# ronghanghu/vit_10b_fsdp_example

Hardware: NVIDIA H100
Metric: vit10b images/sec (device-timed, max over ranks) (higher is better)
Workload: dtype bf16

## Files before the change

vit_10b_fsdp_example_b200/csrc/bindings.cpp:

```cpp
#include <ATen/cuda/CUDAContext.h>
#include <c10/cuda/CUDAGuard.h>
#include <torch/extension.h>

#include <cmath>
#include <optional>
#include <vector>

#include "attention_sm90.h"
#include "comm.h"
#include "elementwise.h"
#include "gemm_sm90.h"

namespace {

using torch::Tensor;
using OptT = std::optional<Tensor>;

inline const __nv_bfloat16* bf16_ptr(const Tensor& t) {
    TORCH_CHECK(t.is_cuda(), "expected a CUDA tensor");
    TORCH_CHECK(t.scalar_type() == at::kBFloat16, "expected a bf16 tensor");
    return reinterpret_cast<const __nv_bfloat16*>(t.data_ptr());
}
inline __nv_bfloat16* bf16_mut(Tensor& t) { return const_cast<__nv_bfloat16*>(bf16_ptr(t)); }
inline float* f32_ptr(const Tensor& t) {
    TORCH_CHECK(t.is_cuda() && t.scalar_type() == at::kFloat, "expected a CUDA fp32 tensor");
    return reinterpret_cast<float*>(t.data_ptr());
}
inline cudaStream_t cur_stream() { return at::cuda::getCurrentCUDAStream().stream(); }

void gemm(Tensor a, int64_t lda, int64_t major_a, Tensor b, int64_t ldb, int64_t major_b, Tensor d, int64_t ldd,
          int64_t M, int64_t N, int64_t K, OptT bias, OptT residual, int64_t ld_res, int64_t res_row_mod, OptT aux_in,
          int64_t ld_aux, OptT aux_out, int64_t ld_aux_out, OptT colsum, int64_t colsum_bi_stride, int64_t act,
          std::vector<int64_t> batch, int64_t block_n, int64_t max_ctas, std::vector<int64_t> ag) {
    c10::cuda::CUDAGuard guard(a.device());
    b200::GemmOperand A, B, D, X;
    A.ptr = bf16_ptr(a), A.ld = lda;
    B.ptr = bf16_ptr(b), B.ld = ldb;
    D.ptr = bf16_ptr(d), D.ld = ldd;
    if (!batch.empty()) {
        TORCH_CHECK(batch.size() == 8, "batch spec must have 8 entries");
        A.nb_inner = B.nb_inner = D.nb_inner = batch[0];
        A.nb_outer = B.nb_outer = D.nb_outer = batch[1];
        A.stride_b_inner = batch[2], A.stride_b_outer = batch[3];
        B.stride_b_inner = batch[4], B.stride_b_outer = batch[5];
        D.stride_b_inner = batch[6], D.stride_b_outer = batch[7];
    }
    b200::GemmEpilogue e;
    if (bias.has_value()) e.bias = bf16_ptr(*bias);
    if (residual.has_value()) e.residual = bf16_ptr(*residual), e.ld_res = ld_res, e.res_row_mod = (int)res_row_mod;
    if (aux_in.has_value()) e.aux_in = bf16_ptr(*aux_in), e.ld_aux = ld_aux;
    if (colsum.has_value()) e.colsum = f32_ptr(*colsum), e.colsum_bi_stride = colsum_bi_stride;
    e.act = static_cast<int>(act);
    if (aux_out.has_value()) {
        X = D;
        X.ptr = bf16_ptr(*aux_out), X.ld = ld_aux_out;
        e.has_aux_out = 1;
    }
    b200::GemmAgFuse fuse;
    if (!ag.empty()) {
        TORCH_CHECK(ag.size() >= 6 && (int64_t)ag.size() == 6 + ag[0] && ag[0] <= 16, "bad AG-fusion spec");
        fuse.world = (int)ag[0], fuse.rank = (int)ag[1], fuse.rows_per_slab = (int)ag[2], fuse.slab_bytes = ag[3];
        fuse.dst = reinterpret_cast<void*>(ag[4]);
        fuse.flags = reinterpret_cast<uint32_t*>(ag[5]);
        for (int64_t r = 0; r < ag[0]; ++r) fuse.peer_src[r] = static_cast<uint64_t>(ag[6 + r]);
    }
    b200::gemm_bf16(A, (int)major_a, B, (int)major_b, D, aux_out.has_value() ? &X : nullptr, (int)M, (int)N, (int)K, e,
                    (int)block_n, (int)max_ctas, cur_stream(), ag.empty() ? nullptr : &fuse);
}

void layernorm_fwd(Tensor x, Tensor gamma, Tensor beta, Tensor y, Tensor mean, Tensor rstd, double eps) {
    c10::cuda::CUDAGuard guard(x.device());
    const int D = (int)x.size(-1);
    const int rows = (int)(x.numel() / D);
    b200::layernorm_fwd(bf16_ptr(x), bf16_ptr(gamma), bf16_ptr(beta), bf16_mut(y), f32_ptr(mean), f32_ptr(rstd), rows,
                        D, (float)eps, cur_stream());
}

void layernorm_bwd(Tensor dy, Tensor x, Tensor gamma, Tensor mean, Tensor rstd, OptT dres, Tensor dx, Tensor dgamma,
                   Tensor dbeta, OptT dxsum) {
    c10::cuda::CUDAGuard guard(x.device());
    const int D = (int)x.size(-1);
    const int rows = (int)(x.numel() / D);
    b200::layernorm_bwd(bf16_ptr(dy), bf16_ptr(x), bf16_ptr(gamma), f32_ptr(mean), f32_ptr(rstd),
                        dres.has_value() ? bf16_ptr(*dres) : nullptr, bf16_mut(dx), f32_ptr(dgamma), f32_ptr(dbeta),
                        dxsum.has_value() ? f32_ptr(*dxsum) : nullptr, rows, D, cur_stream());
}

void softmax_fwd(Tensor s, int64_t rows, int64_t n, int64_t ld, double scale) {
    c10::cuda::CUDAGuard guard(s.device());
    b200::softmax_fwd(bf16_mut(s), rows, (int)n, ld, (float)scale, cur_stream());
}
void softmax_bwd(Tensor dp, Tensor p, int64_t rows, int64_t n, int64_t ld, double scale) {
    c10::cuda::CUDAGuard guard(p.device());
    b200::softmax_bwd(bf16_mut(dp), bf16_ptr(p), rows, (int)n, ld, (float)scale, cur_stream());
}

bool attention_supported(int64_t N, int64_t hd) { return b200::attention_supported((int)N, (int)hd); }

void attention_fwd(Tensor qkv, Tensor out, OptT lse, OptT probs, int64_t B, int64_t N, int64_t H, int64_t hd) {
    c10::cuda::CUDAGuard guard(qkv.device());
    TORCH_CHECK(qkv.dim() == 2 && qkv.stride(1) == 1 && out.is_contiguous(), "attention_fwd: bad layouts");
    TORCH_CHECK(!lse.has_value() || (lse->is_contiguous() && lse->numel() == B * H * N), "attention_fwd: bad lse");
    b200::attention_fwd(bf16_ptr(qkv), qkv.stride(0), bf16_mut(out), lse.has_value() ? f32_ptr(*lse) : nullptr,
                        probs.has_value() ? bf16_mut(*probs) : nullptr, probs.has_value() ? probs->size(2) : 0, (int)B,
                        (int)N, (int)H, (int)hd, cur_stream());
}

void attention_bwd(Tensor qkv, Tensor dout, Tensor out, Tensor lse, Tensor delta, Tensor dqkv, OptT colsum, int64_t B,
                   int64_t N, int64_t H, int64_t hd) {
    c10::cuda::CUDAGuard guard(qkv.device());
    TORCH_CHECK(qkv.dim() == 2 && qkv.stride(1) == 1 && dout.stride(1) == 1 && out.stride(1) == 1 &&
                    dqkv.is_contiguous() && lse.is_contiguous() && delta.is_contiguous(),
                "attention_bwd: bad layouts");
    TORCH_CHECK(lse.numel() == B * H * N && delta.numel() == B * H * N && dqkv.size(1) == 3 * H * hd,
                "attention_bwd: bad shapes");
    b200::attention_bwd(bf16_ptr(qkv), qkv.stride(0), bf16_ptr(dout), dout.stride(0), bf16_ptr(out), out.stride(0),
                        f32_ptr(lse), f32_ptr(delta), bf16_mut(dqkv), (int)B, (int)N, (int)H, (int)hd, cur_stream(),
                        colsum.has_value() ? f32_ptr(*colsum) : nullptr);
}

void cross_entropy(Tensor logits, Tensor target, OptT dlogits, Tensor loss, OptT correct) {
    c10::cuda::CUDAGuard guard(logits.device());
    TORCH_CHECK(target.scalar_type() == at::kLong && target.is_cuda(), "target must be a CUDA int64 tensor");
    const int B = (int)logits.size(0), C = (int)logits.size(1);
    b200::cross_entropy(bf16_ptr(logits), reinterpret_cast<const int64_t*>(target.data_ptr()),
                        dlogits.has_value() ? bf16_mut(*dlogits) : nullptr, f32_ptr(loss),
                        correct.has_value() ? reinterpret_cast<int*>(correct->data_ptr()) : nullptr, B, C,
                        cur_stream());
}

void im2col(Tensor img, Tensor cols, int64_t P) {
    c10::cuda::CUDAGuard guard(img.device());
    TORCH_CHECK(img.is_contiguous() && img.dim() == 4 && img.size(1) == 3, "images must be contiguous [B,3,S,S]");
    const bool is_bf16 = img.scalar_type() == at::kBFloat16;
    TORCH_CHECK(is_bf16 || img.scalar_type() == at::kFloat, "images must be fp32 or bf16");
    b200::im2col(img.data_ptr(), is_bf16, bf16_mut(cols), (int)img.size(0), (int)img.size(2), (int)P,
                 (int)cols.size(1), cur_stream());
}

void gelu_fwd(Tensor u, Tensor g) {
    c10::cuda::CUDAGuard guard(u.device());
    b200::gelu_fwd(bf16_ptr(u), bf16_mut(g), u.numel(), cur_stream());
}
void dropout(Tensor x, Tensor y, double p, int64_t key) {
    c10::cuda::CUDAGuard guard(x.device());
    TORCH_CHECK(x.is_contiguous() && y.is_contiguous() && x.numel() == y.numel(), "dropout: contiguous, same size");
    b200::dropout(bf16_ptr(x), bf16_mut(y), x.numel(), (float)p, (uint64_t)key, cur_stream());
}
void meanpool_fwd(Tensor xn, Tensor pooled, int64_t B, int64_t N) {
    c10::cuda::CUDAGuard guard(xn.device());
    TORCH_CHECK(xn.is_contiguous() && pooled.is_contiguous() && xn.numel() == pooled.numel() * N, "meanpool: bad shapes");
    b200::meanpool_fwd(bf16_ptr(xn), bf16_mut(pooled), (int)B, (int)N, (int)(pooled.numel() / B), cur_stream());
// ... 70 lines not shown
void ce_all_gather(std::vector<int64_t> src_ptrs, std::vector<int64_t> dst_ptrs, std::vector<int64_t> nbytes) {
    TORCH_CHECK(src_ptrs.size() == dst_ptrs.size() && src_ptrs.size() == nbytes.size(), "ce_all_gather: ragged lists");
    cudaStream_t stream = cur_stream();
    for (size_t i = 0; i < src_ptrs.size(); ++i) {
        cudaError_t err = cudaMemcpyAsync(reinterpret_cast<void*>(dst_ptrs[i]), reinterpret_cast<const void*>(src_ptrs[i]),
                                          static_cast<size_t>(nbytes[i]), cudaMemcpyDeviceToDevice, stream);
        TORCH_CHECK(err == cudaSuccess, "ce_all_gather: ", cudaGetErrorString(err));
    }
}
bool make_adam(const OptT& hi, const OptT& lo, const OptT& m, const OptT& v, const std::vector<double>& hyper,
               b200::AdamFuse& a) {
    if (!hi.has_value()) return false;
    TORCH_CHECK(lo.has_value() && m.has_value() && v.has_value() && hyper.size() == 6, "bad fused-AdamW arguments");
    TORCH_CHECK(hi->scalar_type() == at::kBFloat16 && lo->scalar_type() == at::kShort, "hi: bf16, lo: int16");
    a.hi = reinterpret_cast<uint16_t*>(hi->data_ptr());
    a.lo = reinterpret_cast<int16_t*>(lo->data_ptr());
    a.m = f32_ptr(*m);
    a.v = f32_ptr(*v);
    a.lr = (float)hyper[0], a.beta1 = (float)hyper[1], a.beta2 = (float)hyper[2], a.eps = (float)hyper[3];
    a.wd = (float)hyper[4];
    a.inv_bc1 = 1.f / (1.f - powf(a.beta1, (float)hyper[5]));
    a.inv_bc2 = 1.f / (1.f - powf(a.beta2, (float)hyper[5]));
    return true;
}
inline uint32_t* seq_ptr(const OptT& t) {
    if (!t.has_value()) return nullptr;
    TORCH_CHECK(t->is_cuda() && t->scalar_type() == at::kInt, "sequence counters: CUDA int32 tensor");
    return reinterpret_cast<uint32_t*>(t->data_ptr());
}
bool make_sync(const std::vector<int64_t>& sync, const std::vector<int64_t>& flag_ptrs, const OptT& seq_dev,
               const OptT& cta_ctr, b200::CommSync& cs) {
    if (sync.empty()) return false;
    TORCH_CHECK(sync.size() == 5 && seq_dev.has_value() && cta_ctr.has_value(), "bad collective sync arguments");
    cs.flag_ptrs = flag_ptrs;
    cs.rank = (int)sync[0], cs.world = (int)sync[1], cs.slot_ready = (int)sync[2], cs.slot_done = (int)sync[3];
    cs.counter_idx = (int)sync[4];
    cs.seq_dev = seq_ptr(seq_dev);
    cs.cta_ctr = seq_ptr(cta_ctr);
    return true;
}
void reduce_scatter(std::vector<int64_t> peer_ptrs, int64_t mc_ptr, int64_t rank, int64_t world, Tensor out,
                    Tensor seg_table, int64_t total_chunks, bool in_is_bf16, double scale, OptT sumsq_out,
                    int64_t max_ctas, std::vector<int64_t> sync, std::vector<int64_t> flag_ptrs, OptT seq_dev,
                    OptT cta_ctr, OptT hi, OptT lo, OptT m, OptT v, std::vector<double> hyper) {
    c10::cuda::CUDAGuard guard(out.device());
    b200::AdamFuse a;
    const bool fused = make_adam(hi, lo, m, v, hyper, a);
    b200::CommSync cs;
    const bool synced = make_sync(sync, flag_ptrs, seq_dev, cta_ctr, cs);
    b200::reduce_scatter(peer_ptrs, mc_ptr, (int)rank, (int)world, f32_ptr(out), seg_ptr(seg_table),
                         (int)seg_table.size(0), total_chunks, in_is_bf16, (float)scale,
                         sumsq_out.has_value() ? f32_ptr(*sumsq_out) : nullptr, (int)max_ctas, cur_stream(),
                         synced ? &cs : nullptr, fused ? &a : nullptr);
}
void all_reduce_mean(std::vector<int64_t> peer_ptrs, int64_t mc_ptr, int64_t rank, int64_t world, Tensor buf,
                     int64_t max_ctas, std::vector<int64_t> sync, std::vector<int64_t> flag_ptrs, OptT seq_dev,
                     OptT cta_ctr) {
    c10::cuda::CUDAGuard guard(buf.device());
    TORCH_CHECK(buf.scalar_type() == at::kBFloat16 && buf.is_contiguous(), "all_reduce_mean: contiguous bf16 buffer");
    b200::CommSync cs;
    TORCH_CHECK(make_sync(sync, flag_ptrs, seq_dev, cta_ctr, cs), "all_reduce_mean needs the flag protocol");
    b200::all_reduce_mean_bf16(peer_ptrs, mc_ptr, (int)rank, (int)world, buf.numel() * 2, 1.0f / (float)world,
                               (int)max_ctas, cur_stream(), &cs);
}
void signal_barrier(std::vector<int64_t> flag_ptrs, int64_t rank, int64_t world, int64_t slot, int64_t seq,
                    OptT seq_dev) {
    b200::signal_barrier(flag_ptrs, (int)rank, (int)world, (int)slot, (uint32_t)seq, cur_stream(), seq_ptr(seq_dev));
}
void allreduce_scalars(std::vector<int64_t> flag_ptrs, std::vector<int64_t> scratch_ptrs, int64_t rank, int64_t world,
                       int64_t slot, int64_t seq, Tensor vals, int64_t op, OptT seq_dev, int64_t counter_idx) {
    c10::cuda::CUDAGuard guard(vals.device());
    b200::allreduce_scalars(flag_ptrs, scratch_ptrs, (int)rank, (int)world, (int)slot, (uint32_t)seq, f32_ptr(vals),
                            (int)vals.numel(), (int)op, cur_stream(), seq_ptr(seq_dev), (int)counter_idx);
}
int64_t ag_chunk_bytes() { return b200::ag_chunk_bytes(); }
int64_t rs_chunk_elems() { return b200::rs_chunk_elems(); }
int64_t rs_chunk_vecs() { return b200::rs_chunk_vecs(); }

}

PYBIND11_MODULE(TORCH_EXTENSION_NAME, m) {
    m.doc() = "vit_10b_fsdp_example_b200 native sm_90a kernels";
    m.def("gemm", &gemm);
    m.def("layernorm_fwd", &layernorm_fwd);
    m.def("layernorm_bwd", &layernorm_bwd);
    m.def("softmax_fwd", &softmax_fwd);
    m.def("softmax_bwd", &softmax_bwd);
    m.def("attention_fwd", &attention_fwd);
    m.def("attention_supported", &attention_supported);
    m.def("attention_bwd", &attention_bwd);
    m.def("cross_entropy", &cross_entropy);
    m.def("im2col", &im2col);
    m.def("gelu_fwd", &gelu_fwd);
    m.def("dgelu_mul", &dgelu_mul);
    m.def("dropout", &dropout);
    m.def("meanpool_fwd", &meanpool_fwd);
    m.def("meanpool_bwd", &meanpool_bwd);
    m.def("colsum", &colsum);
    m.def("sumsq", &sumsq);
    m.def("adamw_split", &adamw_split);
    m.def("adamw_fp32", &adamw_fp32);
    m.def("split_fp32", &split_fp32);
    m.def("merge_fp32", &merge_fp32);
    m.def("clip_coef", &clip_coef);
    m.def("p2p_all_gather", &p2p_all_gather);
    m.def("ce_all_gather", &ce_all_gather);
    m.def("reduce_scatter", &reduce_scatter);
    m.def("all_reduce_mean", &all_reduce_mean);
    m.def("rs_chunk_vecs", &rs_chunk_vecs);
    m.def("signal_barrier", &signal_barrier);
    m.def("allreduce_scalars", &allreduce_scalars);
    m.def("ag_chunk_bytes", &ag_chunk_bytes);
    m.def("rs_chunk_elems", &rs_chunk_elems);
}
```

vit_10b_fsdp_example_b200/csrc/gemm_sm90.cu:

```cuda
#include <cuda.h>
#include <cuda_runtime.h>
#include <cuda_bf16.h>
#include <cstdint>
#include <cstdio>
#include <cstdlib>
#include <cstring>
#include <mutex>
#include <stdexcept>
#include <string>
#include <algorithm>
#include <unordered_map>

#include "gemm_sm90.h"
#include "ptx.cuh"
#include "wgmma.cuh"

namespace b200 {

namespace {

constexpr int kBlockM = 128;
constexpr int kBlockK = 64;
constexpr int kMmaK = 16;
constexpr int kConsumerWgs = 2;
constexpr int kNumThreads = 384;
constexpr int kEpiThreads = 128;
constexpr int kCdBufs = 4;
constexpr int kCdBufBytes = 64 * 128;

struct KernelParams {
    int M, N, K;
    int batch, nb_inner;
    int m_tiles, n_tiles;
    int n_rot;
    int group_n;
    GemmEpilogue epi;
    GemmAgFuse ag;
};

constexpr int kAgChunkBytes = 16384;

__device__ __forceinline__ uint4 ld_peer_v4(const void* ptr) {
    uint4 r;
    asm volatile("ld.global.L1::no_allocate.v4.u32 {%0, %1, %2, %3}, [%4];"
                 : "=r"(r.x), "=r"(r.y), "=r"(r.z), "=r"(r.w)
                 : "l"(ptr)
                 : "memory");
    return r;
}
__device__ __forceinline__ void red_release_gpu_add(uint32_t* ptr, uint32_t v) {
    asm volatile("red.release.gpu.global.add.u32 [%0], %1;" ::"l"(ptr), "r"(v) : "memory");
}
__device__ __forceinline__ uint32_t ld_acquire_gpu(const uint32_t* ptr) {
    uint32_t v;
    asm volatile("ld.acquire.gpu.global.u32 %0, [%1];" : "=r"(v) : "l"(ptr) : "memory");
    return v;
}
__device__ __forceinline__ void fence_proxy_async_all() { asm volatile("fence.proxy.async;" ::: "memory"); }

__device__ __forceinline__ float erf_as(float z, float& e) {
    const float az = fabsf(z);
    const float t = __frcp_rn(fmaf(0.3275911f, az, 1.0f));
    e = __expf(-az * az);
    float poly = fmaf(1.061405429f, t, -1.453152027f);
    poly = fmaf(poly, t, 1.421413741f);
    poly = fmaf(poly, t, -0.284496736f);
    poly = fmaf(poly, t, 0.254829592f);
    const float y = 1.0f - poly * t * e;
    return copysignf(y, z);
}
__device__ __forceinline__ float gelu_erf(float x) {
    float e;
    return 0.5f * x * (1.0f + erf_as(x * 0.70710678118654752f, e));
}
__device__ __forceinline__ float dgelu_erf(float x) {
    float e;
    const float cdf = 0.5f * (1.0f + erf_as(x * 0.70710678118654752f, e));
    return fmaf(x * 0.3989422804014327f, e, cdf);
}

template <int kMajorA, int kMajorB, int BLOCK_N, int kStages>
__global__ void __launch_bounds__(kNumThreads, 1)
    gemm_bf16_sm90_kernel(const __grid_constant__ CUtensorMap tmap_a, const __grid_constant__ CUtensorMap tmap_b,
                          const __grid_constant__ CUtensorMap tmap_d, const __grid_constant__ CUtensorMap tmap_aux,
                          const KernelParams p) {
    constexpr int kABytes = kBlockM * kBlockK * 2;
    constexpr int kBBytes = BLOCK_N * kBlockK * 2;
    constexpr int kStageBytes = kABytes + kBBytes;
    static_assert(BLOCK_N % 64 == 0 && BLOCK_N <= 256, "epilogue works in 64-column chunks; wgmma N <= 256");
    static_assert(kABytes % 1024 == 0 && kBBytes % 1024 == 0, "swizzle-128B needs 1024 B aligned stages");

    extern __shared__ __align__(1024) uint8_t smem[];
    uint8_t* smem_cd = smem;
    uint8_t* smem_a = smem + kCdBufs * kCdBufBytes;
    uint8_t* smem_b = smem_a + kStages * kABytes;
    uint64_t* full_bar = reinterpret_cast<uint64_t*>(smem_b + kStages * kBBytes);
    uint64_t* empty_bar = full_bar + kStages;

    const uint32_t warp_idx = threadIdx.x / 32;
    const uint32_t lane = lane_id();
    const uint32_t wg = warp_idx / 4;
    if (threadIdx.x == 0 && (smem_u32(smem) & 1023u) != 0) {
        printf("[b200] gemm: dynamic shared memory is not 1024-byte aligned\n");
        __trap();
    }

    if (warp_idx == 0 && elect_one()) {
        prefetch_tmap(&tmap_a);
        prefetch_tmap(&tmap_b);
        prefetch_tmap(&tmap_d);
        if (p.epi.has_aux_out) prefetch_tmap(&tmap_aux);
        for (int i = 0; i < kStages; ++i) {
            mbar_init(&full_bar[i], 1);
            mbar_init(&empty_bar[i], kConsumerWgs * 4);
        }
        fence_mbar_init();
    }
    __syncthreads();

    const int tiles_per_batch = p.m_tiles * p.n_tiles;
    const int total_tiles = tiles_per_batch * p.batch;
    const int num_kb = (p.K + kBlockK - 1) / kBlockK;
    const int kGroupN = p.group_n;

    auto decode_tile = [&](int t, int& b, int& mt, int& nt) {
        b = t / tiles_per_batch;
        const int r = t - b * tiles_per_batch;
        const int per_group = p.m_tiles * kGroupN;
        const int g = r / per_group;
        const int first_n = g * kGroupN;
        const int gsz = min(kGroupN, p.n_tiles - first_n);
        const int in_g = r - g * per_group;
        mt = in_g / gsz;
        nt = first_n + in_g % gsz;
        nt += p.n_rot;
        if (nt >= p.n_tiles) nt -= p.n_tiles;
    };
    const int ag_chunks_per_slab =
        p.ag.world > 1 ? static_cast<int>((p.ag.slab_bytes + kAgChunkBytes - 1) / kAgChunkBytes) : 0;

    if (wg == 0) {
        reg_dealloc<56>();
        if (warp_idx == 0) {
            if (elect_one()) {
                uint32_t stage = 0, phase = 0;
                for (int t = blockIdx.x; t < total_tiles; t += gridDim.x) {
                    int b, mt, nt;
                    decode_tile(t, b, mt, nt);
                    const int bi = b % p.nb_inner, bo = b / p.nb_inner;
                    const int m_idx = mt * kBlockM;
                    const int n_idx = nt * BLOCK_N;
                    if (p.ag.world > 1) {
                        const int last_row = min(n_idx + BLOCK_N, p.N) - 1;
                        if (last_row >= n_idx) {
                            const int s_lo = min(n_idx / p.ag.rows_per_slab, p.ag.world - 1);
                            const int s_hi = min(last_row / p.ag.rows_per_slab, p.ag.world - 1);
                            for (int sl = s_lo; sl <= s_hi; ++sl) {
                                uint32_t spins = 0;
                                while (ld_acquire_gpu(p.ag.flags + sl) < static_cast<uint32_t>(ag_chunks_per_slab)) {
                                    if (++spins > (1u << 26)) {
                                        printf("[b200] AG-fused GEMM: slab %d never arrived (block %d)\n", sl, blockIdx.x);
                                        __trap();
                                    }
                                }
                            }
                            fence_proxy_async_all();
                        }
                    }
                    for (int kb = 0; kb < num_kb; ++kb) {
                        mbar_wait(&empty_bar[stage], phase ^ 1);
                        const int k_idx = kb * kBlockK;
                        uint8_t* sa = smem_a + stage * kABytes;
                        uint8_t* sb = smem_b + stage * kBBytes;
                        mbar_arrive_expect_tx(&full_bar[stage], kStageBytes);
                        if constexpr (kMajorA == 0) {
                            tma_load_4d(&tmap_a, &full_bar[stage], sa, k_idx, m_idx, bi, bo);
                        } else {
#pragma unroll
                            for (int i = 0; i < kBlockM / 64; ++i)
                                tma_load_4d(&tmap_a, &full_bar[stage], sa + i * (64 * kBlockK * 2), m_idx + i * 64,
                                                 k_idx, bi, bo);
                        }
                        if constexpr (kMajorB == 0) {
                            tma_load_4d(&tmap_b, &full_bar[stage], sb, k_idx, n_idx, bi, bo);
                        } else {
#pragma unroll
                            for (int i = 0; i < BLOCK_N / 64; ++i)
                                tma_load_4d(&tmap_b, &full_bar[stage], sb + i * (64 * kBlockK * 2), n_idx + i * 64,
                                                 k_idx, bi, bo);
                        }
                        stage = (stage + 1 == kStages) ? 0 : stage + 1;
                        phase ^= (stage == 0);
                    }
                }
            }
        } else if (warp_idx == 1) {
            if (p.ag.world > 1) {
                const int total_chunks = p.ag.world * ag_chunks_per_slab;
                uint32_t* chunk_counter = p.ag.flags + p.ag.world;
                for (;;) {
                    int c = 0;
                    if (lane == 0) c = static_cast<int>(atomicAdd(chunk_counter, 1u));
                    c = __shfl_sync(0xffffffffu, c, 0);
                    if (c >= total_chunks) break;
                    const int k = c / ag_chunks_per_slab;
                    const int sl = (p.ag.rank + k) % p.ag.world;
                    const int64_t off = static_cast<int64_t>(c - k * ag_chunks_per_slab) * kAgChunkBytes;
                    const int64_t nbytes = min(static_cast<int64_t>(kAgChunkBytes), p.ag.slab_bytes - off);
                    const uint8_t* src = reinterpret_cast<const uint8_t*>(p.ag.peer_src[sl]) + off;
                    uint8_t* dst = static_cast<uint8_t*>(p.ag.dst) + static_cast<int64_t>(sl) * p.ag.slab_bytes + off;
                    const int nvec = static_cast<int>(nbytes / 16);
                    int i = lane;
                    for (; i + 3 * 32 < nvec; i += 4 * 32) {
                        uint4 v[4];
#pragma unroll
                        for (int u = 0; u < 4; ++u) v[u] = ld_peer_v4(src + static_cast<int64_t>(i + u * 32) * 16);
#pragma unroll
                        for (int u = 0; u < 4; ++u) *reinterpret_cast<uint4*>(dst + static_cast<int64_t>(i + u * 32) * 16) = v[u];
                    }
                    for (; i < nvec; i += 32) *reinterpret_cast<uint4*>(dst + static_cast<int64_t>(i) * 16) = ld_peer_v4(src + static_cast<int64_t>(i) * 16);
                    __threadfence();
                    __syncwarp();
                    if (lane == 0) red_release_gpu_add(p.ag.flags + sl, 1);
                }
            }
        }
    } else {
        reg_alloc<224>();
        const uint32_t cw = wg - 1;
        const uint32_t etid = threadIdx.x & 127;
        const uint32_t wrow = (warp_idx & 3) * 16 + lane / 4;
        const uint32_t cpair = (lane & 3) * 2;
        const uint32_t bar_id = 1 + cw;
        uint8_t* const grp_buf = smem_cd + cw * 2 * kCdBufBytes;
        const GemmEpilogue& e = p.epi;
        const bool ext_is_aux = e.act == kActDGelu;
        constexpr uint32_t kLbo = kBlockK * 128;
        constexpr uint32_t kKStepA = kMajorA == 0 ? (kMmaK * 2) : (kMmaK * 128);
        constexpr uint32_t kKStepB = kMajorB == 0 ? (kMmaK * 2) : (kMmaK * 128);
        constexpr uint32_t kSlabA = 64 * kBlockK * 2;
        uint32_t stage = 0, phase = 0;
        uint32_t flip = 0;
        float d[BLOCK_N / 2];

        for (int t = blockIdx.x; t < total_tiles; t += gridDim.x) {
            int b, mt, nt;
            decode_tile(t, b, mt, nt);
            const int bi = b % p.nb_inner, bo = b / p.nb_inner;
            const int m0 = mt * kBlockM + cw * 64;
            const int n0 = nt * BLOCK_N;

            uint32_t prev_stage = 0;
            for (int kb = 0; kb < num_kb; ++kb) {
                mbar_wait(&full_bar[stage], phase);
                const uint32_t a_addr = smem_u32(smem_a + stage * kABytes) + cw * kSlabA;
                const uint32_t b_addr = smem_u32(smem_b + stage * kBBytes);
                wgmma_fence();
#pragma unroll
                for (int k = 0; k < kBlockK / kMmaK; ++k) {
                    const uint64_t da = make_wgmma_desc(a_addr + k * kKStepA, kLbo, 1024, 1);
                    const uint64_t db = make_wgmma_desc(b_addr + k * kKStepB, kLbo, 1024, 1);
                    WgmmaSS<BLOCK_N, kMajorA, kMajorB>::mma(d, da, db, (kb > 0 || k > 0) ? 1u : 0u);
                }
                wgmma_commit();
                if (kb > 0) {
                    wgmma_wait<1>();
                    if (lane == 0) mbar_arrive(&empty_bar[prev_stage]);
                }
                prev_stage = stage;
                stage = (stage + 1 == kStages) ? 0 : stage + 1;
                phase ^= (stage == 0);
            }
            wgmma_wait<0>();
            if (lane == 0) mbar_arrive(&empty_bar[prev_stage]);

            const int row0 = m0 + static_cast<int>(wrow), row1 = row0 + 8;
            const bool row0_ok = row0 < p.M, row1_ok = row1 < p.M;
            const __nv_bfloat16 *ext0 = nullptr, *ext1 = nullptr;
            if (ext_is_aux) {
                ext0 = e.aux_in + static_cast<int64_t>(row0) * e.ld_aux;
                ext1 = e.aux_in + static_cast<int64_t>(row1) * e.ld_aux;
            } else if (e.residual != nullptr) {
                ext0 = e.residual + static_cast<int64_t>(e.res_row_mod > 0 ? row0 % e.res_row_mod : row0) * e.ld_res;
                ext1 = e.residual + static_cast<int64_t>(e.res_row_mod > 0 ? row1 % e.res_row_mod : row1) * e.ld_res;
            }
#pragma unroll
            for (int c = 0; c < BLOCK_N / 64; ++c) {
                const int ncol0 = n0 + c * 64;
                if (ncol0 >= p.N) continue;
                uint8_t* buf0 = grp_buf + (e.has_aux_out ? 0 : (flip & 1)) * kCdBufBytes;
                uint8_t* buf1 = grp_buf + kCdBufBytes;
                if (etid == 0) {
                    if (e.has_aux_out)
                        tma_store_wait_read<0>();
                    else
                        tma_store_wait_read<1>();
                }
                named_bar_sync(bar_id, kEpiThreads);
#pragma unroll
                for (int j = 0; j < 8; ++j) {
                    const int col = ncol0 + j * 8 + static_cast<int>(cpair);
                    const bool c0_ok = col < p.N, c1_ok = col + 1 < p.N;
                    float v[4] = {d[(c * 8 + j) * 4], d[(c * 8 + j) * 4 + 1], d[(c * 8 + j) * 4 + 2], d[(c * 8 + j) * 4 + 3]};
                    uint32_t x0 = 0, x1 = 0;
                    if (ext0 != nullptr && c0_ok) {
                        if (row0_ok) x0 = __ldg(reinterpret_cast<const uint32_t*>(ext0 + col));
                        if (row1_ok) x1 = __ldg(reinterpret_cast<const uint32_t*>(ext1 + col));
                    }
                    if (e.bias != nullptr && c0_ok) {
                        const uint32_t bw = __ldg(reinterpret_cast<const uint32_t*>(e.bias + col));
                        v[0] += bf16_lo(bw), v[1] += bf16_hi(bw), v[2] += bf16_lo(bw), v[3] += bf16_hi(bw);
                    }
                    const uint32_t off0 = wrow * 128 + ((j ^ (wrow & 7)) * 16) + cpair * 2;
                    const uint32_t off1 = off0 + 8 * 128;
                    if (e.has_aux_out) {
                        st_shared_b32(smem_u32(buf1) + off0, pack_bf16x2(v[0], v[1]));
                        st_shared_b32(smem_u32(buf1) + off1, pack_bf16x2(v[2], v[3]));
                    }
                    if (e.act == kActGelu) {
#pragma unroll
                        for (int q = 0; q < 4; ++q) v[q] = gelu_erf(v[q]);
                    } else if (ext_is_aux) {
                        v[0] *= dgelu_erf(bf16_lo(x0)), v[1] *= dgelu_erf(bf16_hi(x0));
                        v[2] *= dgelu_erf(bf16_lo(x1)), v[3] *= dgelu_erf(bf16_hi(x1));
                    }
                    if (e.residual != nullptr && !ext_is_aux) {
                        v[0] += bf16_lo(x0), v[1] += bf16_hi(x0), v[2] += bf16_lo(x1), v[3] += bf16_hi(x1);
                    }
                    if (!(row0_ok && c0_ok)) v[0] = 0.f;
                    if (!(row0_ok && c1_ok)) v[1] = 0.f;
                    if (!(row1_ok && c0_ok)) v[2] = 0.f;
                    if (!(row1_ok && c1_ok)) v[3] = 0.f;
                    st_shared_b32(smem_u32(buf0) + off0, pack_bf16x2(v[0], v[1]));
                    st_shared_b32(smem_u32(buf0) + off1, pack_bf16x2(v[2], v[3]));
                }
                fence_proxy_async_smem();
                named_bar_sync(bar_id, kEpiThreads);
                if (etid == 0) {
                    tma_store_4d(&tmap_d, buf0, ncol0, m0, bi, bo);
                    tma_store_commit();
                    if (e.has_aux_out) {
                        tma_store_4d(&tmap_aux, buf1, ncol0, m0, bi, bo);
                        tma_store_commit();
                    }
                }
                if (e.colsum != nullptr) {
                    const int ccol = etid & 63;
                    const int rhalf = etid >> 6;
                    const int jj = ccol >> 3, within = ccol & 7;
                    float s = 0.f;
#pragma unroll 8
                    for (int r = 0; r < 32; ++r) {
                        const int rr = rhalf * 32 + r;
                        const uint8_t* ptr = buf0 + rr * 128 + ((jj ^ (rr & 7)) * 16) + within * 2;
                        s += __bfloat162float(*reinterpret_cast<const __nv_bfloat16*>(ptr));
                    }
                    if (ncol0 + ccol < p.N)
                        atomicAdd(e.colsum + static_cast<int64_t>(bi) * e.colsum_bi_stride + ncol0 + ccol, s);
                }
                ++flip;
            }
        }
        if (etid == 0) tma_store_wait<0>();
    }
}

using EncodeFn = CUresult (*)(CUtensorMap*, CUtensorMapDataType, cuuint32_t, void*, const cuuint64_t*,
                              const cuuint64_t*, const cuuint32_t*, const cuuint32_t*, CUtensorMapInterleave,
                              CUtensorMapSwizzle, CUtensorMapL2promotion, CUtensorMapFloatOOBfill);

EncodeFn get_encode_fn() {
    static EncodeFn fn = nullptr;
    static std::once_flag once;
    std::call_once(once, [] {
        void* sym = nullptr;
        cudaDriverEntryPointQueryResult qres;
        cudaError_t err = cudaGetDriverEntryPoint("cuTensorMapEncodeTiled", &sym, cudaEnableDefault, &qres);
        if (err != cudaSuccess || qres != cudaDriverEntryPointSuccess || sym == nullptr)
            throw std::runtime_error("cuTensorMapEncodeTiled not available from the driver");
        fn = reinterpret_cast<EncodeFn>(sym);
    });
    return fn;
}

struct TmapKey {
    uint64_t ptr;
    int64_t d[4];
    int64_t s[3];
    int32_t box[2];
    bool operator==(const TmapKey& o) const { return std::memcmp(this, &o, sizeof(TmapKey)) == 0; }
};
struct TmapKeyHash {
    size_t operator()(const TmapKey& k) const {
        const uint64_t* w = reinterpret_cast<const uint64_t*>(&k);
        size_t h = 1469598103934665603ull;
        for (size_t i = 0; i < sizeof(TmapKey) / 8; ++i) h = (h ^ w[i]) * 1099511628211ull;
        return h;
    }
};

CUtensorMap make_tmap(const GemmOperand& op, int64_t inner, int64_t outer, int box_inner, int box_outer,
                      int swizzle_bytes = 128) {
    static std::unordered_map<TmapKey, CUtensorMap, TmapKeyHash> cache;
    static std::mutex mu;
    TmapKey key;
    std::memset(&key, 0, sizeof(key));
    key.ptr = reinterpret_cast<uint64_t>(op.ptr);
    key.d[0] = inner, key.d[1] = outer, key.d[2] = op.nb_inner, key.d[3] = op.nb_outer;
    key.s[0] = op.ld, key.s[1] = op.stride_b_inner, key.s[2] = op.stride_b_outer;
    key.box[0] = box_inner, key.box[1] = box_outer + (swizzle_bytes << 16);
    {
        std::lock_guard<std::mutex> lock(mu);
        auto it = cache.find(key);
        if (it != cache.end()) return it->second;
    }
    if ((reinterpret_cast<uint64_t>(op.ptr) & 15) != 0) throw std::runtime_error("gemm: operand base must be 16 B aligned");
    if ((op.ld * 2) % 16 != 0) throw std::runtime_error("gemm: leading dimension must be a multiple of 8 elements");
    CUtensorMap tm;
    cuuint64_t dims[4] = {static_cast<cuuint64_t>(inner), static_cast<cuuint64_t>(outer),
                          static_cast<cuuint64_t>(op.nb_inner), static_cast<cuuint64_t>(op.nb_outer)};
    const int64_t sbi = op.nb_inner > 1 ? op.stride_b_inner : op.ld * outer;
    const int64_t sbo = op.nb_outer > 1 ? op.stride_b_outer : sbi * op.nb_inner;
    if ((sbi * 2) % 16 != 0 || (sbo * 2) % 16 != 0) throw std::runtime_error("gemm: batch strides must be multiples of 8 elements");
    cuuint64_t strides[3] = {static_cast<cuuint64_t>(op.ld * 2), static_cast<cuuint64_t>(sbi * 2),
                             static_cast<cuuint64_t>(sbo * 2)};
    cuuint32_t box[4] = {static_cast<cuuint32_t>(box_inner), static_cast<cuuint32_t>(box_outer), 1, 1};
    cuuint32_t estr[4] = {1, 1, 1, 1};
    CUresult res = get_encode_fn()(&tm, CU_TENSOR_MAP_DATA_TYPE_BFLOAT16, 4, const_cast<void*>(op.ptr), dims, strides,
                                   box, estr, CU_TENSOR_MAP_INTERLEAVE_NONE,
                                   swizzle_bytes == 128 ? CU_TENSOR_MAP_SWIZZLE_128B
                                   : swizzle_bytes == 64 ? CU_TENSOR_MAP_SWIZZLE_64B
                                                         : CU_TENSOR_MAP_SWIZZLE_32B,
                                   CU_TENSOR_MAP_L2_PROMOTION_L2_256B, CU_TENSOR_MAP_FLOAT_OOB_FILL_NONE);
    if (res != CUDA_SUCCESS) {
        char msg[256];
        snprintf(msg, sizeof(msg),
                 "cuTensorMapEncodeTiled failed (%d): dims=(%lld,%lld,%lld,%lld) ld=%lld box=(%d,%d)", (int)res,
                 (long long)inner, (long long)outer, (long long)op.nb_inner, (long long)op.nb_outer, (long long)op.ld,
                 box_inner, box_outer);
        throw std::runtime_error(msg);
    }
    std::lock_guard<std::mutex> lock(mu);
    if (cache.size() > 4096) cache.clear();
    cache.emplace(key, tm);
    return tm;
}

int num_sms() {
    static int n = 0;
    if (n == 0) {
        int dev = 0;
        cudaGetDevice(&dev);
        cudaDeviceGetAttribute(&n, cudaDevAttrMultiProcessorCount, dev);
    }
    return n;
}

template <int kMajorA, int kMajorB, int BLOCK_N, int kStages>
void launch(const GemmOperand& A, const GemmOperand& B, const GemmOperand& D, const GemmOperand* aux, int M, int N,
            int K, const GemmEpilogue& epi, int max_ctas, cudaStream_t stream, const GemmAgFuse* ag) {
    constexpr int kSmem = kCdBufs * kCdBufBytes + kStages * (kBlockM + BLOCK_N) * kBlockK * 2 + 2 * kStages * 8;
    static_assert(kSmem <= 232448, "shared memory budget exceeded (227 KB per block on sm_90)");
    auto kern = gemm_bf16_sm90_kernel<kMajorA, kMajorB, BLOCK_N, kStages>;
    static bool attr_set = false;
    if (!attr_set) {
        cudaError_t err = cudaFuncSetAttribute(kern, cudaFuncAttributeMaxDynamicSharedMemorySize, kSmem);
        if (err != cudaSuccess) throw std::runtime_error(std::string("cudaFuncSetAttribute: ") + cudaGetErrorString(err));
        attr_set = true;
    }
    CUtensorMap ta = kMajorA == 0 ? make_tmap(A, K, M, kBlockK, kBlockM) : make_tmap(A, M, K, 64, kBlockK);
    CUtensorMap tb = kMajorB == 0 ? make_tmap(B, K, N, kBlockK, BLOCK_N) : make_tmap(B, N, K, 64, kBlockK);
    CUtensorMap td = make_tmap(D, N, M, 64, 64);
    CUtensorMap tx = (epi.has_aux_out && aux != nullptr) ? make_tmap(*aux, N, M, 64, 64) : td;

    KernelParams p;
    p.M = M, p.N = N, p.K = K;
    p.batch = static_cast<int>(D.nb_inner * D.nb_outer);
    p.nb_inner = static_cast<int>(D.nb_inner);
    p.m_tiles = (M + kBlockM - 1) / kBlockM;
    p.n_tiles = (N + BLOCK_N - 1) / BLOCK_N;
    p.epi = epi;
    p.n_rot = 0;
    p.group_n = 2048 / BLOCK_N;
    if (ag != nullptr && ag->world > 1) {
        if (kMajorB != 0 || p.batch != 1) throw std::runtime_error("gemm: AG fusion needs a K-major, un-batched B");
        if (static_cast<int64_t>(ag->rows_per_slab) * K * 2 != ag->slab_bytes || ag->slab_bytes % 16 != 0)
            throw std::runtime_error("gemm: AG fusion needs whole rows per slab");
        p.ag = *ag;
        p.n_rot = static_cast<int>((static_cast<int64_t>(ag->rank) * ag->rows_per_slab) / BLOCK_N) % p.n_tiles;
        cudaMemsetAsync(ag->flags, 0, sizeof(uint32_t) * (ag->world + 1), stream);
    }
    const int64_t total = static_cast<int64_t>(p.m_tiles) * p.n_tiles * p.batch;
    int sms = num_sms();
    if (max_ctas > 0 && max_ctas < sms) sms = max_ctas;
    const int ctas = static_cast<int>(std::max<int64_t>(1, std::min<int64_t>(total, sms)));
    kern<<<ctas, kNumThreads, kSmem, stream>>>(ta, tb, td, tx, p);
    cudaError_t err = cudaGetLastError();
    if (err != cudaSuccess) throw std::runtime_error(std::string("gemm launch failed: ") + cudaGetErrorString(err));
}

}

CUtensorMap make_tensor_map_4d(const GemmOperand& op, int64_t inner, int64_t outer, int box_inner, int box_outer,
                               int swizzle_bytes) {
    return make_tmap(op, inner, outer, box_inner, box_outer, swizzle_bytes);
}

void gemm_bf16(const GemmOperand& A, int major_a, const GemmOperand& B, int major_b, const GemmOperand& D,
               const GemmOperand* aux_out, int M, int N, int K, const GemmEpilogue& epi, int block_n, int max_ctas,
               cudaStream_t stream, const GemmAgFuse* ag) {
    if (N % 8 != 0 && (epi.residual || epi.aux_in))
        throw std::runtime_error("gemm: N must be a multiple of 8 when residual/aux_in are used");
    if (epi.act == kActDGelu && (epi.residual != nullptr || epi.aux_in == nullptr))
        throw std::runtime_error("gemm: dGELU epilogue needs aux_in and cannot be combined with a residual");
    if (D.nb_inner * D.nb_outer > 1 && (epi.bias || epi.residual || epi.aux_in))
        throw std::runtime_error("gemm: bias/residual/aux_in are not supported for batched problems");
    if (block_n == 0) block_n = (N > 128) ? 256 : 128;
#define B200_DISPATCH(MA, MB, BN, ST)                                                             \
    if (major_a == MA && major_b == MB && block_n == BN) {                                        \
        launch<MA, MB, BN, ST>(A, B, D, aux_out, M, N, K, epi, max_ctas, stream, ag);             \
        return;                                                                                   \
    }
    B200_DISPATCH(0, 0, 256, 4)
    B200_DISPATCH(0, 1, 256, 4)
    B200_DISPATCH(1, 1, 256, 4)
    B200_DISPATCH(1, 0, 256, 4)
    B200_DISPATCH(0, 0, 128, 6)
    B200_DISPATCH(0, 1, 128, 6)
    B200_DISPATCH(1, 1, 128, 6)
    B200_DISPATCH(1, 0, 128, 6)
#undef B200_DISPATCH
    throw std::runtime_error("gemm: unsupported (major_a, major_b, block_n) combination");
}

}
```

vit_10b_fsdp_example_b200/csrc/gemm_sm90.h:

```cpp
#pragma once
#include <cuda.h>
#include <cuda_runtime.h>
#include <cuda_bf16.h>
#include <cstdint>

namespace b200 {

enum GemmAct : int { kActNone = 0, kActGelu = 1, kActDGelu = 2 };

struct GemmOperand {
    const void* ptr = nullptr;
    int64_t ld = 0;
    int64_t nb_inner = 1, stride_b_inner = 0;
    int64_t nb_outer = 1, stride_b_outer = 0;
};

struct GemmEpilogue {
    const __nv_bfloat16* bias = nullptr;
    const __nv_bfloat16* residual = nullptr;
    const __nv_bfloat16* aux_in = nullptr;
    float* colsum = nullptr;
    int64_t ld_res = 0;
    int64_t ld_aux = 0;
    int64_t colsum_bi_stride = 0;
    int res_row_mod = 0;
    int act = kActNone;
    int has_aux_out = 0;
};

struct GemmAgFuse {
    int world = 0;
    int rank = 0;
    int rows_per_slab = 0;
    int64_t slab_bytes = 0;
    uint64_t peer_src[16] = {0};
    void* dst = nullptr;
    uint32_t* flags = nullptr;
};

void gemm_bf16(const GemmOperand& A, int major_a, const GemmOperand& B, int major_b, const GemmOperand& D,
               const GemmOperand* aux_out, int M, int N, int K, const GemmEpilogue& epi, int block_n, int max_ctas,
               cudaStream_t stream, const GemmAgFuse* ag = nullptr);

CUtensorMap make_tensor_map_4d(const GemmOperand& op, int64_t inner, int64_t outer, int box_inner, int box_outer,
                               int swizzle_bytes);

}
```

vit_10b_fsdp_example_b200/csrc/ptx.cuh:

```cuda
#pragma once
#include <cuda_runtime.h>
#include <cuda_bf16.h>
#include <cstdint>
#include <cstdio>

namespace b200 {

#ifndef B200_SPIN_LIMIT
#define B200_SPIN_LIMIT (1u << 28)
#endif

__device__ __forceinline__ uint32_t smem_u32(const void* p) {
    return static_cast<uint32_t>(__cvta_generic_to_shared(p));
}

__device__ __forceinline__ uint32_t lane_id() {
    uint32_t l;
    asm volatile("mov.u32 %0, %%laneid;" : "=r"(l));
    return l;
}

__device__ __forceinline__ uint32_t cluster_ctarank() {
    uint32_t r;
    asm volatile("mov.u32 %0, %%cluster_ctarank;" : "=r"(r));
// ... 13 lines not shown
}

__device__ __forceinline__ void cluster_arrive() {
    asm volatile("barrier.cluster.arrive.release.aligned;" ::: "memory");
}
__device__ __forceinline__ void cluster_wait() {
    asm volatile("barrier.cluster.wait.acquire.aligned;" ::: "memory");
}
__device__ __forceinline__ void cluster_sync() {
    cluster_arrive();
    cluster_wait();
}

__device__ __forceinline__ void mbar_init(uint64_t* bar, uint32_t count) {
    asm volatile("mbarrier.init.shared::cta.b64 [%0], %1;" ::"r"(smem_u32(bar)), "r"(count) : "memory");
}

__device__ __forceinline__ void fence_mbar_init() {
    asm volatile("fence.mbarrier_init.release.cluster;" ::: "memory");
}

__device__ __forceinline__ void fence_proxy_async_smem() {
    asm volatile("fence.proxy.async.shared::cta;" ::: "memory");
}

__device__ __forceinline__ void mbar_arrive_expect_tx(uint64_t* bar, uint32_t bytes) {
    asm volatile("mbarrier.arrive.expect_tx.shared::cta.b64 _, [%0], %1;" ::"r"(smem_u32(bar)), "r"(bytes)
                 : "memory");
}

__device__ __forceinline__ void mbar_arrive(uint64_t* bar) {
    asm volatile("mbarrier.arrive.shared::cta.b64 _, [%0];" ::"r"(smem_u32(bar)) : "memory");
}

__device__ __forceinline__ void mbar_arrive_cluster(uint64_t* bar, uint32_t cta) {
    asm volatile(
        "{\n\t"
        ".reg .b32 raddr;\n\t"
        "mapa.shared::cluster.u32 raddr, %0, %1;\n\t"
        "mbarrier.arrive.shared::cluster.b64 _, [raddr];\n\t"
        "}\n" ::"r"(smem_u32(bar)),
        "r"(cta)
        : "memory");
}

__device__ __forceinline__ bool mbar_try_wait(uint64_t* bar, uint32_t phase) {
    uint32_t ok;
    asm volatile(
        "{\n\t"
        ".reg .pred P1;\n\t"
        "mbarrier.try_wait.parity.shared::cta.b64 P1, [%1], %2;\n\t"
        "selp.u32 %0, 1, 0, P1;\n\t"
        "}\n"
        : "=r"(ok)
        : "r"(smem_u32(bar)), "r"(phase)
        : "memory");
    return ok != 0;
}

__device__ __forceinline__ void mbar_wait(uint64_t* bar, uint32_t phase) {
    uint32_t spins = 0;
    while (!mbar_try_wait(bar, phase)) {
        if (++spins > B200_SPIN_LIMIT) {
            printf("[b200] mbarrier timeout: block %d thread %d bar %u phase %u\n", blockIdx.x, threadIdx.x,
                   smem_u32(bar), phase);
            __trap();
        }
    }
}

__device__ __forceinline__ void prefetch_tmap(const void* tmap) {
    asm volatile("prefetch.tensormap [%0];" ::"l"(reinterpret_cast<uint64_t>(tmap)) : "memory");
}

__device__ __forceinline__ void tma_load_4d(const void* tmap, uint64_t* bar, void* smem, int c0, int c1, int c2,
                                            int c3) {
    asm volatile(
        "cp.async.bulk.tensor.4d.shared::cluster.global.mbarrier::complete_tx::bytes"
        " [%0], [%1, {%3, %4, %5, %6}], [%2];" ::"r"(smem_u32(smem)),
        "l"(reinterpret_cast<uint64_t>(tmap)), "r"(smem_u32(bar)), "r"(c0), "r"(c1), "r"(c2), "r"(c3)
        : "memory");
}

__device__ __forceinline__ void tma_store_4d(const void* tmap, const void* smem, int c0, int c1, int c2, int c3) {
    asm volatile(
        "cp.async.bulk.tensor.4d.global.shared::cta.bulk_group [%0, {%2, %3, %4, %5}], [%1];" ::"l"(
            reinterpret_cast<uint64_t>(tmap)),
        "r"(smem_u32(smem)), "r"(c0), "r"(c1), "r"(c2), "r"(c3)
        : "memory");
}

__device__ __forceinline__ void tma_store_commit() { asm volatile("cp.async.bulk.commit_group;" ::: "memory"); }

template <int N>
__device__ __forceinline__ void tma_store_wait_read() {
    asm volatile("cp.async.bulk.wait_group.read %0;" ::"n"(N) : "memory");
}
template <int N>
__device__ __forceinline__ void tma_store_wait() {
    asm volatile("cp.async.bulk.wait_group %0;" ::"n"(N) : "memory");
}

template <int N>
__device__ __forceinline__ void reg_dealloc() {
    asm volatile("setmaxnreg.dec.sync.aligned.u32 %0;" ::"n"(N));
}
template <int N>
__device__ __forceinline__ void reg_alloc() {
    asm volatile("setmaxnreg.inc.sync.aligned.u32 %0;" ::"n"(N));
}

__device__ __forceinline__ uint32_t pack_bf16x2(float lo, float hi) {
    __nv_bfloat162 v = __floats2bfloat162_rn(lo, hi);
    return *reinterpret_cast<uint32_t*>(&v);
}
__device__ __forceinline__ float bf16_lo(uint32_t v) { return __uint_as_float(v << 16); }
__device__ __forceinline__ float bf16_hi(uint32_t v) { return __uint_as_float(v & 0xFFFF0000u); }

__device__ __forceinline__ void named_bar_sync(uint32_t id, uint32_t nthreads) {
    asm volatile("bar.sync %0, %1;" ::"r"(id), "r"(nthreads) : "memory");
}

__device__ __forceinline__ void st_shared_b32(uint32_t addr, uint32_t a) {
    asm volatile("st.shared.b32 [%0], %1;" ::"r"(addr), "r"(a) : "memory");
}

__device__ __forceinline__ void st_shared_v4(uint32_t addr, uint32_t a, uint32_t b, uint32_t c, uint32_t d) {
    asm volatile("st.shared.v4.b32 [%0], {%1, %2, %3, %4};" ::"r"(addr), "r"(a), "r"(b), "r"(c), "r"(d) : "memory");
}

}
```

Baseline: 125.5.

## Launch GEMM as 2-CTA clusters multicasting shared B tiles via TMA

Pairs CTAs into clusters of two that handle adjacent M tiles with the same N tile. Each CTA loads half of the B tile and multicasts it to both CTAs, and empty barriers count arrivals from both CTAs so a slot is released cluster-wide. The aim is to halve L2-to-SMEM traffic for B and raise effective arithmetic intensity. In exchange, the two CTAs are coupled in lockstep, the grid is sized by cluster occupancy, and BLOCK_N must now be a multiple of 128.

```diff
diff --git a/vit_10b_fsdp_example_b200/csrc/bindings.cpp b/vit_10b_fsdp_example_b200/csrc/bindings.cpp
--- a/vit_10b_fsdp_example_b200/csrc/bindings.cpp
+++ b/vit_10b_fsdp_example_b200/csrc/bindings.cpp
@@ -68,6 +68,8 @@
                     (int)block_n, (int)max_ctas, cur_stream(), ag.empty() ? nullptr : &fuse);
 }
 
+int64_t gemm_max_active_clusters(int64_t block_n) { return b200::gemm_max_active_clusters((int)block_n); }
+
 void layernorm_fwd(Tensor x, Tensor gamma, Tensor beta, Tensor y, Tensor mean, Tensor rstd, double eps) {
     c10::cuda::CUDAGuard guard(x.device());
     const int D = (int)x.size(-1);
@@ -304,6 +306,7 @@
 PYBIND11_MODULE(TORCH_EXTENSION_NAME, m) {
     m.doc() = "vit_10b_fsdp_example_b200 native sm_90a kernels";
     m.def("gemm", &gemm);
+    m.def("gemm_max_active_clusters", &gemm_max_active_clusters);
     m.def("layernorm_fwd", &layernorm_fwd);
     m.def("layernorm_bwd", &layernorm_bwd);
     m.def("softmax_fwd", &softmax_fwd);
diff --git a/vit_10b_fsdp_example_b200/csrc/gemm_sm90.cu b/vit_10b_fsdp_example_b200/csrc/gemm_sm90.cu
--- a/vit_10b_fsdp_example_b200/csrc/gemm_sm90.cu
+++ b/vit_10b_fsdp_example_b200/csrc/gemm_sm90.cu
@@ -23,6 +23,7 @@
 constexpr int kBlockK = 64;
 constexpr int kMmaK = 16;
 constexpr int kConsumerWgs = 2;
+constexpr int kClusterSize = 2;
 constexpr int kNumThreads = 384;
 constexpr int kEpiThreads = 128;
 constexpr int kCdBufs = 4;
@@ -32,6 +33,7 @@
     int M, N, K;
     int batch, nb_inner;
     int m_tiles, n_tiles;
+    int m_pairs;
     int n_rot;
     int group_n;
     GemmEpilogue epi;
@@ -39,6 +41,9 @@
 };
 
 constexpr int kAgChunkBytes = 16384;
+
+__device__ __forceinline__ int cluster_idx() { return static_cast<int>(blockIdx.x) / kClusterSize; }
+__device__ __forceinline__ int num_clusters() { return static_cast<int>(gridDim.x) / kClusterSize; }
 
 __device__ __forceinline__ uint4 ld_peer_v4(const void* ptr) {
     uint4 r;
@@ -87,7 +92,9 @@
     constexpr int kABytes = kBlockM * kBlockK * 2;
     constexpr int kBBytes = BLOCK_N * kBlockK * 2;
     constexpr int kStageBytes = kABytes + kBBytes;
-    static_assert(BLOCK_N % 64 == 0 && BLOCK_N <= 256, "epilogue works in 64-column chunks; wgmma N <= 256");
+    constexpr int kBHalf = BLOCK_N / kClusterSize;
+    static_assert(BLOCK_N % 128 == 0 && BLOCK_N <= 256,
+                  "epilogue works in 64-column chunks, a B half is whole 64-row boxes; wgmma N <= 256");
     static_assert(kABytes % 1024 == 0 && kBBytes % 1024 == 0, "swizzle-128B needs 1024 B aligned stages");
 
     extern __shared__ __align__(1024) uint8_t smem[];
@@ -112,26 +119,26 @@
         if (p.epi.has_aux_out) prefetch_tmap(&tmap_aux);
         for (int i = 0; i < kStages; ++i) {
             mbar_init(&full_bar[i], 1);
-            mbar_init(&empty_bar[i], kConsumerWgs * 4);
+            mbar_init(&empty_bar[i], kClusterSize * kConsumerWgs * 4);
         }
         fence_mbar_init();
     }
-    __syncthreads();
-
-    const int tiles_per_batch = p.m_tiles * p.n_tiles;
-    const int total_tiles = tiles_per_batch * p.batch;
+    cluster_sync();
+
+    const int pairs_per_batch = p.m_pairs * p.n_tiles;
+    const int total_pairs = pairs_per_batch * p.batch;
     const int num_kb = (p.K + kBlockK - 1) / kBlockK;
     const int kGroupN = p.group_n;
 
     auto decode_tile = [&](int t, int& b, int& mt, int& nt) {
-        b = t / tiles_per_batch;
-        const int r = t - b * tiles_per_batch;
-        const int per_group = p.m_tiles * kGroupN;
+        b = t / pairs_per_batch;
+        const int r = t - b * pairs_per_batch;
+        const int per_group = p.m_pairs * kGroupN;
         const int g = r / per_group;
         const int first_n = g * kGroupN;
         const int gsz = min(kGroupN, p.n_tiles - first_n);
         const int in_g = r - g * per_group;
-        mt = in_g / gsz;
+        mt = (in_g / gsz) * kClusterSize + static_cast<int>(cluster_ctarank());
         nt = first_n + in_g % gsz;
         nt += p.n_rot;
         if (nt >= p.n_tiles) nt -= p.n_tiles;
@@ -144,7 +151,7 @@
         if (warp_idx == 0) {
             if (elect_one()) {
                 uint32_t stage = 0, phase = 0;
-                for (int t = blockIdx.x; t < total_tiles; t += gridDim.x) {
+                for (int t = cluster_idx(); t < total_pairs; t += num_clusters()) {
                     int b, mt, nt;
                     decode_tile(t, b, mt, nt);
                     const int bi = b % p.nb_inner, bo = b / p.nb_inner;
@@ -181,13 +188,17 @@
                                 tma_load_4d(&tmap_a, &full_bar[stage], sa + i * (64 * kBlockK * 2), m_idx + i * 64,
                                                  k_idx, bi, bo);
                         }
+                        constexpr uint16_t kBothCtas = (1u << kClusterSize) - 1;
+                        const uint32_t r = cluster_ctarank();
+                        const int n_half = n_idx + static_cast<int>(r) * kBHalf;
+                        uint8_t* sb_half = sb + r * (kBHalf * kBlockK * 2);
                         if constexpr (kMajorB == 0) {
-                            tma_load_4d(&tmap_b, &full_bar[stage], sb, k_idx, n_idx, bi, bo);
+                            tma_load_4d_multicast(&tmap_b, &full_bar[stage], sb_half, k_idx, n_half, bi, bo, kBothCtas);
                         } else {
 #pragma unroll
-                            for (int i = 0; i < BLOCK_N / 64; ++i)
-                                tma_load_4d(&tmap_b, &full_bar[stage], sb + i * (64 * kBlockK * 2), n_idx + i * 64,
-                                                 k_idx, bi, bo);
+                            for (int i = 0; i < kBHalf / 64; ++i)
+                                tma_load_4d_multicast(&tmap_b, &full_bar[stage], sb_half + i * (64 * kBlockK * 2),
+                                                      n_half + i * 64, k_idx, bi, bo, kBothCtas);
                         }
                         stage = (stage + 1 == kStages) ? 0 : stage + 1;
                         phase ^= (stage == 0);
@@ -242,8 +253,12 @@
         uint32_t stage = 0, phase = 0;
         uint32_t flip = 0;
         float d[BLOCK_N / 2];
-
-        for (int t = blockIdx.x; t < total_tiles; t += gridDim.x) {
+        auto release_slot = [&](uint32_t s) {
+            mbar_arrive(&empty_bar[s]);
+            mbar_arrive_cluster(&empty_bar[s], cluster_ctarank() ^ 1u);
+        };
+
+        for (int t = cluster_idx(); t < total_pairs; t += num_clusters()) {
             int b, mt, nt;
             decode_tile(t, b, mt, nt);
             const int bi = b % p.nb_inner, bo = b / p.nb_inner;
@@ -265,14 +280,14 @@
                 wgmma_commit();
                 if (kb > 0) {
                     wgmma_wait<1>();
-                    if (lane == 0) mbar_arrive(&empty_bar[prev_stage]);
+                    if (lane == 0) release_slot(prev_stage);
                 }
                 prev_stage = stage;
                 stage = (stage + 1 == kStages) ? 0 : stage + 1;
                 phase ^= (stage == 0);
             }
             wgmma_wait<0>();
-            if (lane == 0) mbar_arrive(&empty_bar[prev_stage]);
+            if (lane == 0) release_slot(prev_stage);
 
             const int row0 = m0 + static_cast<int>(wrow), row1 = row0 + 8;
             const bool row0_ok = row0 < p.M, row1_ok = row1 < p.M;
@@ -363,6 +378,8 @@
         }
         if (etid == 0) tma_store_wait<0>();
     }
+    __syncwarp();
+    cluster_sync();
 }
 
 using EncodeFn = CUresult (*)(CUtensorMap*, CUtensorMapDataType, cuuint32_t, void*, const cuuint64_t*,
@@ -456,20 +473,50 @@
     return n;
 }
 
+constexpr int smem_bytes(int block_n, int stages) {
+    return kCdBufs * kCdBufBytes + stages * (kBlockM + block_n) * kBlockK * 2 + 2 * stages * 8;
+}
+
+cudaLaunchConfig_t cluster_config(int smem, cudaStream_t stream, cudaLaunchAttribute* attr) {
+    attr->id = cudaLaunchAttributeClusterDimension;
+    attr->val.clusterDim.x = kClusterSize, attr->val.clusterDim.y = 1, attr->val.clusterDim.z = 1;
+    cudaLaunchConfig_t cfg = {};
+    cfg.blockDim = dim3(kNumThreads);
+    cfg.dynamicSmemBytes = smem;
+    cfg.stream = stream;
+    cfg.attrs = attr;
+    cfg.numAttrs = 1;
+    return cfg;
+}
+
+template <int kMajorA, int kMajorB, int BLOCK_N, int kStages>
+int max_clusters() {
+    static int n = 0;
+    if (n == 0) {
+        constexpr int kSmem = smem_bytes(BLOCK_N, kStages);
+        auto kern = gemm_bf16_sm90_kernel<kMajorA, kMajorB, BLOCK_N, kStages>;
+        cudaError_t err = cudaFuncSetAttribute(kern, cudaFuncAttributeMaxDynamicSharedMemorySize, kSmem);
+        if (err != cudaSuccess) throw std::runtime_error(std::string("cudaFuncSetAttribute: ") + cudaGetErrorString(err));
+        cudaLaunchAttribute attr;
+        cudaLaunchConfig_t cfg = cluster_config(kSmem, nullptr, &attr);
+        cfg.gridDim = dim3(num_sms() / kClusterSize * kClusterSize);
+        int c = 0;
+        err = cudaOccupancyMaxActiveClusters(&c, kern, &cfg);
+        if (err != cudaSuccess || c < 1)
+            throw std::runtime_error(std::string("gemm: no cluster of 2 CTAs fits: ") + cudaGetErrorString(err));
+        n = c;
+    }
+    return n;
+}
+
 template <int kMajorA, int kMajorB, int BLOCK_N, int kStages>
 void launch(const GemmOperand& A, const GemmOperand& B, const GemmOperand& D, const GemmOperand* aux, int M, int N,
             int K, const GemmEpilogue& epi, int max_ctas, cudaStream_t stream, const GemmAgFuse* ag) {
-    constexpr int kSmem = kCdBufs * kCdBufBytes + kStages * (kBlockM + BLOCK_N) * kBlockK * 2 + 2 * kStages * 8;
+    constexpr int kSmem = smem_bytes(BLOCK_N, kStages);
     static_assert(kSmem <= 232448, "shared memory budget exceeded (227 KB per block on sm_90)");
-    auto kern = gemm_bf16_sm90_kernel<kMajorA, kMajorB, BLOCK_N, kStages>;
-    static bool attr_set = false;
-    if (!attr_set) {
-        cudaError_t err = cudaFuncSetAttribute(kern, cudaFuncAttributeMaxDynamicSharedMemorySize, kSmem);
-        if (err != cudaSuccess) throw std::runtime_error(std::string("cudaFuncSetAttribute: ") + cudaGetErrorString(err));
-        attr_set = true;
-    }
+    const int slots = max_clusters<kMajorA, kMajorB, BLOCK_N, kStages>();
     CUtensorMap ta = kMajorA == 0 ? make_tmap(A, K, M, kBlockK, kBlockM) : make_tmap(A, M, K, 64, kBlockK);
-    CUtensorMap tb = kMajorB == 0 ? make_tmap(B, K, N, kBlockK, BLOCK_N) : make_tmap(B, N, K, 64, kBlockK);
+    CUtensorMap tb = kMajorB == 0 ? make_tmap(B, K, N, kBlockK, BLOCK_N / kClusterSize) : make_tmap(B, N, K, 64, kBlockK);
     CUtensorMap td = make_tmap(D, N, M, 64, 64);
     CUtensorMap tx = (epi.has_aux_out && aux != nullptr) ? make_tmap(*aux, N, M, 64, 64) : td;
 
@@ -478,6 +525,7 @@
     p.batch = static_cast<int>(D.nb_inner * D.nb_outer);
     p.nb_inner = static_cast<int>(D.nb_inner);
     p.m_tiles = (M + kBlockM - 1) / kBlockM;
+    p.m_pairs = (p.m_tiles + kClusterSize - 1) / kClusterSize;
     p.n_tiles = (N + BLOCK_N - 1) / BLOCK_N;
     p.epi = epi;
     p.n_rot = 0;
@@ -490,12 +538,15 @@
         p.n_rot = static_cast<int>((static_cast<int64_t>(ag->rank) * ag->rows_per_slab) / BLOCK_N) % p.n_tiles;
         cudaMemsetAsync(ag->flags, 0, sizeof(uint32_t) * (ag->world + 1), stream);
     }
-    const int64_t total = static_cast<int64_t>(p.m_tiles) * p.n_tiles * p.batch;
-    int sms = num_sms();
-    if (max_ctas > 0 && max_ctas < sms) sms = max_ctas;
-    const int ctas = static_cast<int>(std::max<int64_t>(1, std::min<int64_t>(total, sms)));
-    kern<<<ctas, kNumThreads, kSmem, stream>>>(ta, tb, td, tx, p);
-    cudaError_t err = cudaGetLastError();
+    const int64_t total_pairs = static_cast<int64_t>(p.m_pairs) * p.n_tiles * p.batch;
+    int clusters = slots;
+    if (max_ctas > 0) clusters = std::min(clusters, max_ctas / kClusterSize);
+    clusters = static_cast<int>(std::max<int64_t>(1, std::min<int64_t>(total_pairs, clusters)));
+    cudaLaunchAttribute attr;
+    cudaLaunchConfig_t cfg = cluster_config(kSmem, stream, &attr);
+    cfg.gridDim = dim3(clusters * kClusterSize);
+    cudaError_t err =
+        cudaLaunchKernelEx(&cfg, gemm_bf16_sm90_kernel<kMajorA, kMajorB, BLOCK_N, kStages>, ta, tb, td, tx, p);
     if (err != cudaSuccess) throw std::runtime_error(std::string("gemm launch failed: ") + cudaGetErrorString(err));
 }
 
@@ -533,4 +584,8 @@
     throw std::runtime_error("gemm: unsupported (major_a, major_b, block_n) combination");
 }
 
-}
+int gemm_max_active_clusters(int block_n) {
+    return block_n == 128 ? max_clusters<0, 0, 128, 6>() : max_clusters<0, 0, 256, 4>();
+}
+
+}
diff --git a/vit_10b_fsdp_example_b200/csrc/gemm_sm90.h b/vit_10b_fsdp_example_b200/csrc/gemm_sm90.h
--- a/vit_10b_fsdp_example_b200/csrc/gemm_sm90.h
+++ b/vit_10b_fsdp_example_b200/csrc/gemm_sm90.h
@@ -42,6 +42,8 @@
                const GemmOperand* aux_out, int M, int N, int K, const GemmEpilogue& epi, int block_n, int max_ctas,
                cudaStream_t stream, const GemmAgFuse* ag = nullptr);
 
+int gemm_max_active_clusters(int block_n);
+
 CUtensorMap make_tensor_map_4d(const GemmOperand& op, int64_t inner, int64_t outer, int box_inner, int box_outer,
                                int swizzle_bytes);
 
diff --git a/vit_10b_fsdp_example_b200/csrc/ptx.cuh b/vit_10b_fsdp_example_b200/csrc/ptx.cuh
--- a/vit_10b_fsdp_example_b200/csrc/ptx.cuh
+++ b/vit_10b_fsdp_example_b200/csrc/ptx.cuh
@@ -119,6 +119,15 @@
         : "memory");
 }
 
+__device__ __forceinline__ void tma_load_4d_multicast(const void* tmap, uint64_t* bar, void* smem, int c0, int c1,
+                                                      int c2, int c3, uint16_t cta_mask) {
+    asm volatile(
+        "cp.async.bulk.tensor.4d.shared::cluster.global.mbarrier::complete_tx::bytes.multicast::cluster"
+        " [%0], [%1, {%3, %4, %5, %6}], [%2], %7;" ::"r"(smem_u32(smem)),
+        "l"(reinterpret_cast<uint64_t>(tmap)), "r"(smem_u32(bar)), "r"(c0), "r"(c1), "r"(c2), "r"(c3), "h"(cta_mask)
+        : "memory");
+}
+
 __device__ __forceinline__ void tma_store_4d(const void* tmap, const void* smem, int c0, int c1, int c2, int c3) {
     asm volatile(
         "cp.async.bulk.tensor.4d.global.shared::cta.bulk_group [%0, {%2, %3, %4, %5}], [%1];" ::"l"(
```

New measurement: 125.5, median of 6. No clear change (+0.0%).
